# DavidHuji/CapDec

Hardware: AMD Instinct MI355X
Metric: captions/sec (whole node), COCO-val 5k, prefix_len=10 beam=5, 1/2/4/8 GPUs (higher is better)
Workload: dtype f32 (operands split into 2 fp16 planes, 3 fp16 MFMAs per product, fp32 accumulate); 1 GPU; COCO-val-5k-shaped: 5000 x 512-d synthetic CLIP embeddings in total (sharded over the ranks) -> normalise -> TransformerMapper(8 layers) -> GPT-2 small KV-cached beam-5 decode, prefix_len 10, entry_length 67, hot-init seeded weights (never emit the stop id: all 67 steps run); captions_per_gpu=5000, beam=5, parallelism=caption-shard dp1

## Files before the change

### capdec_amd/csrc/bf16x3.h

```cpp
#pragma once
#include <hip/hip_runtime.h>
#include <stdint.h>

namespace capdec {

typedef __bf16 bf16x8 __attribute__((ext_vector_type(8)));
typedef __bf16 bf16x4 __attribute__((ext_vector_type(4)));

constexpr int X3_BK = 16;
constexpr int X3_ROW_B = 32;
constexpr int X3_TILE_ROWS = 128;
constexpr int X3_PLANE_B = X3_TILE_ROWS * X3_ROW_B;
constexpr int X3_BLOCK_B = 3 * X3_PLANE_B;

__device__ __forceinline__ void split3(const float4 v, bf16x4 &h, bf16x4 &m, bf16x4 &l) {
    const float a[4] = {v.x, v.y, v.z, v.w};
#pragma unroll
    for (int e = 0; e < 4; ++e) {
        const __bf16 hh = (__bf16)a[e];
        const float r1 = a[e] - (float)hh;
        const __bf16 mm = (__bf16)r1;
        const float r2 = r1 - (float)mm;
        h[e] = hh;
        m[e] = mm;
        l[e] = (__bf16)r2;
    }
}

__device__ __forceinline__ int x3_group_offset(int r, int quad) {
    return r * X3_ROW_B + (((quad >> 1) ^ ((r >> 3) & 1)) << 4) + ((quad & 1) << 3);
}

typedef _Float16 f16x8 __attribute__((ext_vector_type(8)));
typedef _Float16 f16x4 __attribute__((ext_vector_type(4)));
enum PackFmt { PK_BF16X3 = 0, PK_F16X2 = 1, PK_BF16X1 = 2, PK_F16X1 = 3 };
constexpr int H2_BLOCK_B = 2 * X3_PLANE_B;
constexpr float H2_LO_SCALE = 2048.0f;

static __device__ unsigned int g_h2_saturated;
#define CAPDEC_SAT_ACCESSOR(fn)                                                                            \
    unsigned long long fn(bool reset) {                                                                    \
        unsigned int v = 0;                                                                                \
        if (hipMemcpyFromSymbol(&v, HIP_SYMBOL(g_h2_saturated), sizeof(v)) != hipSuccess) return 0;        \
        if (reset && v) { const unsigned int z = 0; (void)hipMemcpyToSymbol(HIP_SYMBOL(g_h2_saturated), &z, sizeof(z)); } \
        return v;                                                                                          \
    }
__device__ __forceinline__ float h2_clamp_count(const float4 v) {
    const float m = __builtin_fmaxf(__builtin_fmaxf(__builtin_fabsf(v.x), __builtin_fabsf(v.y)),
                                    __builtin_fmaxf(__builtin_fabsf(v.z), __builtin_fabsf(v.w)));
    if (m > 65504.f) atomicAdd(&g_h2_saturated, 1u);
    return m;
}
__device__ __forceinline__ float h2_clamp(float a) {
    return a != a ? a : __builtin_fminf(__builtin_fmaxf(a, -65504.f), 65504.f);
}

__device__ __forceinline__ void split2h(const float4 v, f16x4 &h, f16x4 &l) {
    const float a[4] = {v.x, v.y, v.z, v.w};
    (void)h2_clamp_count(v);
#pragma unroll
    for (int e = 0; e < 4; ++e) {
        const float c = h2_clamp(a[e]);
        const _Float16 hh = __builtin_fabsf(c) < 0x1p-14f ? (_Float16)0.f : (_Float16)c;
        const float r = c - (float)hh;
        h[e] = hh;
        l[e] = (_Float16)(r * H2_LO_SCALE);
    }
}

__host__ __device__ __forceinline__ int pk_planes(int fmt) {
    return fmt == PK_F16X2 ? 2 : (fmt == PK_BF16X1 || fmt == PK_F16X1) ? 1 : 3;
}

__device__ __forceinline__ void x3_store_quad(char *packed, int nk, int row, int ks, int quad, const float4 v,
                                              int fmt = PK_BF16X3) {
    if (fmt == PK_BF16X1 || fmt == PK_F16X1) {
        char *p = packed + ((size_t)(row >> 7) * nk + ks) * X3_PLANE_B + x3_group_offset(row & 127, quad);
        if (fmt == PK_BF16X1) {
            bf16x4 h;
            h[0] = (__bf16)v.x; h[1] = (__bf16)v.y; h[2] = (__bf16)v.z; h[3] = (__bf16)v.w;
            *reinterpret_cast<bf16x4 *>(p) = h;
        } else {
            f16x4 h;
            (void)h2_clamp_count(v);
            h[0] = (_Float16)h2_clamp(v.x);
            h[1] = (_Float16)h2_clamp(v.y);
            h[2] = (_Float16)h2_clamp(v.z);
            h[3] = (_Float16)h2_clamp(v.w);
            *reinterpret_cast<f16x4 *>(p) = h;
        }
        return;
    }
    if (fmt == PK_F16X2) {
        f16x4 h, l;
        split2h(v, h, l);
        char *p = packed + ((size_t)(row >> 7) * nk + ks) * H2_BLOCK_B + x3_group_offset(row & 127, quad);
        *reinterpret_cast<f16x4 *>(p) = h;
        *reinterpret_cast<f16x4 *>(p + X3_PLANE_B) = l;
        return;
    }
    bf16x4 h, m, l;
    split3(v, h, m, l);
    char *p = packed + ((size_t)(row >> 7) * nk + ks) * X3_BLOCK_B + x3_group_offset(row & 127, quad);
    *reinterpret_cast<bf16x4 *>(p) = h;
    *reinterpret_cast<bf16x4 *>(p + X3_PLANE_B) = m;
    *reinterpret_cast<bf16x4 *>(p + 2 * X3_PLANE_B) = l;
}

__device__ __forceinline__ float4 x3_load_quad(const char *packed, int nk, int row, int ks, int quad, int fmt) {
    if (fmt == PK_F16X2) {
        const char *p = packed + ((size_t)(row >> 7) * nk + ks) * H2_BLOCK_B + x3_group_offset(row & 127, quad);
        const f16x4 h = *reinterpret_cast<const f16x4 *>(p), l = *reinterpret_cast<const f16x4 *>(p + X3_PLANE_B);
        return make_float4((float)h[0] + (float)l[0] * (1.0f / H2_LO_SCALE), (float)h[1] + (float)l[1] * (1.0f / H2_LO_SCALE),
                           (float)h[2] + (float)l[2] * (1.0f / H2_LO_SCALE), (float)h[3] + (float)l[3] * (1.0f / H2_LO_SCALE));
    }
    const char *p = packed + ((size_t)(row >> 7) * nk + ks) * X3_PLANE_B + x3_group_offset(row & 127, quad);
    if (fmt == PK_F16X1) {
        const f16x4 h = *reinterpret_cast<const f16x4 *>(p);
        return make_float4((float)h[0], (float)h[1], (float)h[2], (float)h[3]);
    }
    const bf16x4 h = *reinterpret_cast<const bf16x4 *>(p);
    return make_float4((float)h[0], (float)h[1], (float)h[2], (float)h[3]);
}

inline size_t x3_packed_bytes(int rows, int K, int fmt = PK_BF16X3) {
    return (size_t)((rows + X3_TILE_ROWS - 1) / X3_TILE_ROWS) * X3_TILE_ROWS * K * pk_planes(fmt) * sizeof(uint16_t);
}

}
```

### capdec_amd/csrc/elementwise.hip

```cpp
#include "bf16x3.h"
#include "common.h"

namespace capdec {

constexpr int LN_MAXV = 4;
__global__ __launch_bounds__(256) void layernorm_kernel(const float *__restrict__ x, int ldx,
                                                        const float *__restrict__ w, const float *__restrict__ b,
                                                        float eps, float *__restrict__ y, int ldy, int rows, int d) {
    const int lane = threadIdx.x & 63;
    const int row = blockIdx.x * 4 + (threadIdx.x >> 6);
    if (row >= rows) return;
    const float *xr = x + (size_t)row * ldx;
    const int nv = d >> 2;
    float4 v[LN_MAXV];
    float s = 0.f;
#pragma unroll
    for (int i = 0; i < LN_MAXV; ++i) {
        const int idx = lane + 64 * i;
        if (idx < nv) {
            v[i] = reinterpret_cast<const float4 *>(xr)[idx];
            s += (v[i].x + v[i].y) + (v[i].z + v[i].w);
        } else {
            v[i] = make_float4(0.f, 0.f, 0.f, 0.f);
        }
    }
    const float mean = wave_sum(s) / (float)d;
    float q = 0.f;
#pragma unroll
    for (int i = 0; i < LN_MAXV; ++i) {
        const int idx = lane + 64 * i;
        if (idx < nv) {
            const float a = v[i].x - mean, bb = v[i].y - mean, c = v[i].z - mean, e = v[i].w - mean;
            q += (a * a + bb * bb) + (c * c + e * e);
        }
    }
    const float rstd = 1.0f / sqrtf(wave_sum(q) / (float)d + eps);
    float *yr = y + (size_t)row * ldy;
#pragma unroll
    for (int i = 0; i < LN_MAXV; ++i) {
        const int idx = lane + 64 * i;
        if (idx < nv) {
            const float4 ww = reinterpret_cast<const float4 *>(w)[idx];
            const float4 bb = reinterpret_cast<const float4 *>(b)[idx];
            float4 o;
            o.x = (v[i].x - mean) * rstd * ww.x + bb.x;
            o.y = (v[i].y - mean) * rstd * ww.y + bb.y;
            o.z = (v[i].z - mean) * rstd * ww.z + bb.z;
            o.w = (v[i].w - mean) * rstd * ww.w + bb.w;
            reinterpret_cast<float4 *>(yr)[idx] = o;
        }
    }
}

int launch_layernorm(hipStream_t st, const float *x, int ldx, const float *w, const float *b, float eps, float *y,
                     int ldy, int rows, int d) {
    CAPDEC_CHECK(d % 4 == 0 && d <= 256 * LN_MAXV && ldx % 4 == 0 && ldy % 4 == 0, "layernorm: unsupported width");
    if (rows <= 0) return 0;
    hipLaunchKernelGGL(layernorm_kernel, dim3((rows + 3) / 4), dim3(256), 0, st, x, ldx, w, b, eps, y, ldy, rows, d);
    CAPDEC_HIP(hipGetLastError());
    return 0;
}

template <int LN_RPW>
__global__ __launch_bounds__(256) void layernorm_packed_kernel(const float *__restrict__ x, int ldx,
                                                               const float *__restrict__ w, const float *__restrict__ b,
                                                               float eps, char *__restrict__ packed, int rows, int d,
                                                               int fmt) {
    const int lane = threadIdx.x & 63, wave = threadIdx.x >> 6;
    const int nv = d >> 2, nk = d / X3_BK;
    const int row0 = blockIdx.x * 4 * LN_RPW + wave;
    if (row0 >= rows) return;
    float4 ww[LN_MAXV], bb[LN_MAXV];
#pragma unroll
    for (int i = 0; i < LN_MAXV; ++i) {
        const int idx = lane + 64 * i;
        ww[i] = idx < nv ? reinterpret_cast<const float4 *>(w)[idx] : make_float4(0.f, 0.f, 0.f, 0.f);
        bb[i] = idx < nv ? reinterpret_cast<const float4 *>(b)[idx] : make_float4(0.f, 0.f, 0.f, 0.f);
    }
    float4 v[LN_MAXV], nx[LN_MAXV];
#define LN_LOAD(dst, r)                                                                              \
    _Pragma("unroll") for (int i = 0; i < LN_MAXV; ++i) {                                            \
        const int idx = lane + 64 * i;                                                               \
        dst[i] = (idx < nv && (r) < rows) ? reinterpret_cast<const float4 *>(x + (size_t)(r) * ldx)[idx] \
                                          : make_float4(0.f, 0.f, 0.f, 0.f);                         \
    }
    LN_LOAD(nx, row0)
#pragma unroll
    for (int rr = 0; rr < LN_RPW; ++rr) {
        const int row = row0 + 4 * rr;
        if (row >= rows) break;
#pragma unroll
        for (int i = 0; i < LN_MAXV; ++i) v[i] = nx[i];
        if (rr + 1 < LN_RPW) { LN_LOAD(nx, row + 4) }
        float s = 0.f;
#pragma unroll
        for (int i = 0; i < LN_MAXV; ++i) s += (v[i].x + v[i].y) + (v[i].z + v[i].w);
        const float mean = wave_sum(s) / (float)d;
        float q = 0.f;
#pragma unroll
        for (int i = 0; i < LN_MAXV; ++i) {
            const int idx = lane + 64 * i;
            if (idx < nv) {
                const float a = v[i].x - mean, b2 = v[i].y - mean, c = v[i].z - mean, e = v[i].w - mean;
                q += (a * a + b2 * b2) + (c * c + e * e);
            }
        }
        const float rstd = 1.0f / sqrtf(wave_sum(q) / (float)d + eps);
#pragma unroll
        for (int i = 0; i < LN_MAXV; ++i) {
            const int idx = lane + 64 * i;
            if (idx < nv) {
                float4 o;
                o.x = (v[i].x - mean) * rstd * ww[i].x + bb[i].x;
                o.y = (v[i].y - mean) * rstd * ww[i].y + bb[i].y;
                o.z = (v[i].z - mean) * rstd * ww[i].z + bb[i].z;
                o.w = (v[i].w - mean) * rstd * ww[i].w + bb[i].w;
                x3_store_quad(packed, nk, row, idx >> 2, idx & 3, o, fmt);
            }
        }
    }
#undef LN_LOAD
}

int launch_layernorm_packed(hipStream_t st, const float *x, int ldx, const float *w, const float *b, float eps,
                            void *packed, int rows, int d, int fmt) {
    CAPDEC_CHECK(d % 16 == 0 && d <= 256 * LN_MAXV && ldx % 4 == 0, "layernorm_packed: unsupported width");
    if (rows <= 0) return 0;
    if (rows >= 16384)
        hipLaunchKernelGGL(layernorm_packed_kernel<4>, dim3((rows + 15) / 16), dim3(256), 0, st, x, ldx, w, b, eps,
                           (char *)packed, rows, d, fmt);
    else
        hipLaunchKernelGGL(layernorm_packed_kernel<1>, dim3((rows + 3) / 4), dim3(256), 0, st, x, ldx, w, b, eps,
                           (char *)packed, rows, d, fmt);
    CAPDEC_HIP(hipGetLastError());
    return 0;
}

template <int LN_RPW>
__global__ __launch_bounds__(256) void l2norm_rows_kernel(const float *__restrict__ x, char *__restrict__ packed,
                                                          float *__restrict__ y, int rows, int d, int fmt,
                                                          int *__restrict__ row_bad, int *__restrict__ any_bad) {
    const int lane = threadIdx.x & 63, wave = threadIdx.x >> 6;
    const int nv = d >> 2, nk = d / X3_BK;
    const int row0 = blockIdx.x * 4 * LN_RPW + wave;
    if (row0 >= rows) return;
    float4 v[LN_MAXV], nx[LN_MAXV];
#define L2_LOAD(dst, r)                                                                              \
    _Pragma("unroll") for (int i = 0; i < LN_MAXV; ++i) {                                            \
        const int idx = lane + 64 * i;                                                               \
        dst[i] = (idx < nv && (r) < rows) ? reinterpret_cast<const float4 *>(x + (size_t)(r) * d)[idx] \
                                          : make_float4(0.f, 0.f, 0.f, 0.f);                         \
    }
    L2_LOAD(nx, row0)
#pragma unroll
    for (int rr = 0; rr < LN_RPW; ++rr) {
        const int row = row0 + 4 * rr;
        if (row >= rows) break;
#pragma unroll
        for (int i = 0; i < LN_MAXV; ++i) v[i] = nx[i];
        if (rr + 1 < LN_RPW) { L2_LOAD(nx, row + 4) }
        float q = 0.f, big = 0.f;
#pragma unroll
        for (int i = 0; i < LN_MAXV; ++i) {
            q += (v[i].x * v[i].x + v[i].y * v[i].y) + (v[i].z * v[i].z + v[i].w * v[i].w);
            const float a = __builtin_fabsf(v[i].x), b = __builtin_fabsf(v[i].y), c = __builtin_fabsf(v[i].z),
                        e = __builtin_fabsf(v[i].w);
            big = (a <= 3.402823466e38f && b <= 3.402823466e38f && c <= 3.402823466e38f && e <= 3.402823466e38f) ? big : 1.f;
        }
        const bool bad = wave_max(big) != 0.f;
        const float den = fmaxf(sqrtf(wave_sum(q)), 1e-12f);
        if (lane == 0) {
            if (row_bad) row_bad[row] = bad ? 1 : 0;
            if (bad && any_bad) atomicOr(any_bad, 1);
        }
#pragma unroll
        for (int i = 0; i < LN_MAXV; ++i) {
            const int idx = lane + 64 * i;
            if (idx < nv) {
                const float4 o = bad ? make_float4(0.f, 0.f, 0.f, 0.f)
                                     : make_float4(v[i].x / den, v[i].y / den, v[i].z / den, v[i].w / den);
                if (packed) x3_store_quad(packed, nk, row, idx >> 2, idx & 3, o, fmt);
                else reinterpret_cast<float4 *>(y + (size_t)row * d)[idx] = o;
            }
        }
    }
#undef L2_LOAD
}

int launch_l2norm_rows(hipStream_t st, const float *x, void *packed, float *y, int rows, int d, int fmt, int *row_bad,
                       int *any_bad) {
    CAPDEC_CHECK(d % 4 == 0 && d <= 256 * LN_MAXV && (!packed || d % 16 == 0), "l2norm_rows: unsupported width");
    CAPDEC_CHECK((packed != nullptr) != (y != nullptr), "l2norm_rows: exactly one output form");
    if (rows <= 0) return 0;
    if (rows >= 16384)
        hipLaunchKernelGGL(l2norm_rows_kernel<4>, dim3((rows + 15) / 16), dim3(256), 0, st, x, (char *)packed, y, rows, d, fmt,
                           row_bad, any_bad);
    else
        hipLaunchKernelGGL(l2norm_rows_kernel<1>, dim3((rows + 3) / 4), dim3(256), 0, st, x, (char *)packed, y, rows, d, fmt,
                           row_bad, any_bad);
    CAPDEC_HIP(hipGetLastError());
    return 0;
}

__global__ void embed_tokens_kernel(const int *__restrict__ tok, const float *__restrict__ wte,
                                    const float *__restrict__ wpe_row, float *__restrict__ h, int rows, int nv,
                                    const int *__restrict__ cmap, int beam) {
    const int i = blockIdx.x * blockDim.x + threadIdx.x;
    if (i >= rows * nv) return;
    const int row = i / nv, c = i - row * nv;
    const int srow = cmap ? cmap[row / beam] * beam + row % beam : row;
    const float4 a = reinterpret_cast<const float4 *>(wte + (size_t)tok[srow] * nv * 4)[c];
    const float4 p = reinterpret_cast<const float4 *>(wpe_row)[c];
    reinterpret_cast<float4 *>(h)[i] = make_float4(a.x + p.x, a.y + p.y, a.z + p.z, a.w + p.w);
}
int launch_embed_tokens(hipStream_t st, const int *tok, const float *wte, const float *wpe_row, float *h, int rows,
                        int d, const int *cmap, int beam) {
    if (rows <= 0) return 0;
    const int n = rows * (d / 4);
    hipLaunchKernelGGL(embed_tokens_kernel, dim3((n + 255) / 256), dim3(256), 0, st, tok, wte, wpe_row, h, rows,
                       d / 4, cmap, beam);
    CAPDEC_HIP(hipGetLastError());
    return 0;
}

__global__ void embed_prefix_kernel(const float *__restrict__ prefix, const float *__restrict__ wpe,
                                    float *__restrict__ h, int n, int P, int pos0, int nv) {
    const int i = blockIdx.x * blockDim.x + threadIdx.x;
    if (i >= n * P * nv) return;
    const int c = i % nv, p = (i / nv) % P;
    const float4 a = reinterpret_cast<const float4 *>(prefix)[i];
    const float4 w = reinterpret_cast<const float4 *>(wpe + (size_t)(pos0 + p) * nv * 4)[c];
    reinterpret_cast<float4 *>(h)[i] = make_float4(a.x + w.x, a.y + w.y, a.z + w.z, a.w + w.w);
}
int launch_embed_prefix(hipStream_t st, const float *prefix, const float *wpe, float *h, int n, int P, int pos0,
                        int d) {
    const int tot = n * P * (d / 4);
    if (tot <= 0) return 0;
    hipLaunchKernelGGL(embed_prefix_kernel, dim3((tot + 255) / 256), dim3(256), 0, st, prefix, wpe, h, n, P, pos0,
                       d / 4);
    CAPDEC_HIP(hipGetLastError());
    return 0;
}

__global__ void gather_rows_kernel(const float *__restrict__ table, const int *__restrict__ ids,
                                   float *__restrict__ out, int rows, int nv) {
    const int i = blockIdx.x * blockDim.x + threadIdx.x;
    if (i >= rows * nv) return;
    const int row = i / nv, c = i - row * nv;
    reinterpret_cast<float4 *>(out)[i] = reinterpret_cast<const float4 *>(table + (size_t)ids[row] * nv * 4)[c];
}
int launch_gather_rows(hipStream_t st, const float *table, const int *ids, float *out, int rows, int d) {
    if (rows <= 0) return 0;
    const int n = rows * (d / 4);
    hipLaunchKernelGGL(gather_rows_kernel, dim3((n + 255) / 256), dim3(256), 0, st, table, ids, out, rows, d / 4);
    CAPDEC_HIP(hipGetLastError());
    return 0;
}

__global__ __launch_bounds__(256) void normalize_prefix_kernel(const float *__restrict__ x, int n, int dim,
                                                               int normalize, const float *__restrict__ offset,
                                                               float *__restrict__ out) {
    const int lane = threadIdx.x & 63;
    const int row = blockIdx.x * 4 + (threadIdx.x >> 6);
    if (row >= n) return;
    const float *xr = x + (size_t)row * dim;
    float s = 0.f;
    for (int i = lane; i < dim; i += 64) s += xr[i] * xr[i];
    const float nrm = sqrtf(wave_sum(s));
    for (int i = lane; i < dim; i += 64) {
        float v = xr[i];
        if (normalize) v = v / nrm;
        if (offset) v += offset[i];
        out[(size_t)row * dim + i] = v;
    }
}
int launch_normalize_prefix(hipStream_t st, const float *x, int n, int dim, int normalize, const float *offset,
                            float *out) {
    if (n <= 0) return 0;
    hipLaunchKernelGGL(normalize_prefix_kernel, dim3((n + 3) / 4), dim3(256), 0, st, x, n, dim, normalize, offset,
                       out);
    CAPDEC_HIP(hipGetLastError());
    return 0;
}

__device__ __forceinline__ float u01(uint32_t x) { return ((float)(x >> 8) + 0.5f) * (1.0f / 16777216.0f); }
__device__ __forceinline__ float philox_normal(uint64_t seed, uint64_t idx, uint32_t stream) {
    uint32_t o[4];
    philox4x32((uint32_t)idx, (uint32_t)(idx >> 32), stream, 0u, (uint32_t)seed, (uint32_t)(seed >> 32), o);
    const float r = sqrtf(-2.0f * logf(u01(o[0])));
    return r * cosf(6.283185307179586f * u01(o[1]));
}
__device__ __forceinline__ float philox_uniform(uint64_t seed, uint64_t idx, uint32_t stream) {
    uint32_t o[4];
    philox4x32((uint32_t)idx, (uint32_t)(idx >> 32), stream, 0u, (uint32_t)seed, (uint32_t)(seed >> 32), o);
    return ((float)(o[0] >> 8)) * (1.0f / 16777216.0f);
}

__global__ __launch_bounds__(256) void noise_inject_kernel(const float *__restrict__ x, int n, int dim, float std,
                                                           const float *__restrict__ offset, int uniform,
                                                           int dont_norm, uint64_t seed,
                                                           const float *__restrict__ noise,
                                                           const float *__restrict__ u, float *__restrict__ out) {
    const int lane = threadIdx.x & 63;
    const int row = blockIdx.x * 4 + (threadIdx.x >> 6);
    if (row >= n) return;
    const float *xr = x + (size_t)row * dim;
    float inv1 = 1.f;
    if (!dont_norm) {
        float s = 0.f;
        for (int i = lane; i < dim; i += 64) s += xr[i] * xr[i];
        inv1 = 1.0f / fmaxf(sqrtf(wave_sum(s)), 1e-12f);
    }
    float nscale = std;
    if (uniform) {
        float s = 0.f;
        for (int i = lane; i < dim; i += 64) {
            const float g = noise ? noise[(size_t)row * dim + i] : philox_normal(seed, (uint64_t)row * dim + i, 0u);
            s += g * g;
        }
        const float gn = fmaxf(sqrtf(wave_sum(s)), 1e-12f);
        const float uu = u ? u[row] : philox_uniform(seed, (uint64_t)row, 1u);
        nscale = powf(uu, 1.0f / (float)dim) * std / gn;
    }
    float s2 = 0.f;
    for (int i = lane; i < dim; i += 64) {
        const float g = noise ? noise[(size_t)row * dim + i] : philox_normal(seed, (uint64_t)row * dim + i, 0u);
        float v = (dont_norm ? xr[i] : xr[i] * inv1);
        v = v + g * nscale;
        if (offset) v += offset[i];
        out[(size_t)row * dim + i] = v;
        s2 += v * v;
    }
    const float inv2 = 1.0f / fmaxf(sqrtf(wave_sum(s2)), 1e-12f);
    for (int i = lane; i < dim; i += 64) out[(size_t)row * dim + i] *= inv2;
}
int launch_noise_inject(hipStream_t st, const float *x, int n, int dim, float variance, const float *offset,
                        int uniform, int dont_norm, uint64_t seed, const float *noise, const float *u, float *out) {
    if (n <= 0) return 0;
    if (variance == 0.0f) {
        if (out != x) CAPDEC_HIP(hipMemcpyAsync(out, x, (size_t)n * dim * sizeof(float), hipMemcpyDeviceToDevice, st));
        return 0;
    }
    CAPDEC_CHECK(out != x, "noise_inject: in-place not supported");
    hipLaunchKernelGGL(noise_inject_kernel, dim3((n + 3) / 4), dim3(256), 0, st, x, n, dim, sqrtf(variance), offset,
                       uniform, dont_norm, seed, noise, u, out);
    CAPDEC_HIP(hipGetLastError());
    return 0;
}

__global__ void tmapper_concat_kernel(const float *__restrict__ lin, const float *__restrict__ pc,
                                      float *__restrict__ seq, int n, int clip_len, int P, int nv) {
    const int i = blockIdx.x * blockDim.x + threadIdx.x;
    const int S = clip_len + P;
    if (i >= n * S * nv) return;
    const int c = i % nv, s = (i / nv) % S, cap = i / (nv * S);
    float4 v;
    if (s < clip_len) v = reinterpret_cast<const float4 *>(lin)[((size_t)cap * clip_len + s) * nv + c];
    else v = reinterpret_cast<const float4 *>(pc)[(size_t)(s - clip_len) * nv + c];
    reinterpret_cast<float4 *>(seq)[i] = v;
}
int launch_tmapper_concat(hipStream_t st, const float *lin, const float *prefix_const, float *seq, int n,
                          int clip_len, int P, int d) {
    const int tot = n * (clip_len + P) * (d / 4);
    if (tot <= 0) return 0;
    hipLaunchKernelGGL(tmapper_concat_kernel, dim3((tot + 255) / 256), dim3(256), 0, st, lin, prefix_const, seq, n,
                       clip_len, P, d / 4);
    CAPDEC_HIP(hipGetLastError());
    return 0;
}
__global__ void tmapper_take_kernel(const float *__restrict__ seq, float *__restrict__ out, int n, int clip_len,
                                    int P, int nv) {
    const int i = blockIdx.x * blockDim.x + threadIdx.x;
    if (i >= n * P * nv) return;
    const int c = i % nv, p = (i / nv) % P, cap = i / (nv * P);
    reinterpret_cast<float4 *>(out)[i] =
        reinterpret_cast<const float4 *>(seq)[((size_t)cap * (clip_len + P) + clip_len + p) * nv + c];
}
int launch_tmapper_take(hipStream_t st, const float *seq, float *out, int n, int clip_len, int P, int d) {
    const int tot = n * P * (d / 4);
    if (tot <= 0) return 0;
    hipLaunchKernelGGL(tmapper_take_kernel, dim3((tot + 255) / 256), dim3(256), 0, st, seq, out, n, clip_len, P,
                       d / 4);
    CAPDEC_HIP(hipGetLastError());
    return 0;
}

__global__ void transpose_kernel(const float *__restrict__ in, float *__restrict__ out, int rows, int cols) {
    __shared__ float tile[32][33];
    const int bx = blockIdx.x * 32, by = blockIdx.y * 32;
    const int tx = threadIdx.x & 31, ty = threadIdx.x >> 5;
    for (int j = ty; j < 32; j += 8) {
        const int r = by + j, c = bx + tx;
        if (r < rows && c < cols) tile[j][tx] = in[(size_t)r * cols + c];
    }
    __syncthreads();
    for (int j = ty; j < 32; j += 8) {
        const int c = bx + j, r = by + tx;
        if (r < rows && c < cols) out[(size_t)c * rows + r] = tile[tx][j];
    }
}
int launch_transpose(hipStream_t st, const float *in, float *out, int rows, int cols) {
    hipLaunchKernelGGL(transpose_kernel, dim3((cols + 31) / 32, (rows + 31) / 32), dim3(256), 0, st, in, out, rows,
                       cols);
    CAPDEC_HIP(hipGetLastError());
    return 0;
}

__global__ void clip_text_embed_kernel(const int *__restrict__ tokens, const float *__restrict__ tok_emb,
                                       const float *__restrict__ pos_emb, float *__restrict__ h, int n, int L, int P,
                                       const int *__restrict__ perm, int nv) {
    const int i = blockIdx.x * blockDim.x + threadIdx.x;
    if (i >= n * P * nv) return;
    const int c = i % nv, row = i / nv, t = row % P, cap = row / P;
    const int tok = tokens[(size_t)(perm ? perm[cap] : cap) * L + t];
    const float4 a = reinterpret_cast<const float4 *>(tok_emb + (size_t)tok * nv * 4)[c];
    const float4 p = reinterpret_cast<const float4 *>(pos_emb + (size_t)t * nv * 4)[c];
    reinterpret_cast<float4 *>(h)[i] = make_float4(a.x + p.x, a.y + p.y, a.z + p.z, a.w + p.w);
}
int launch_clip_text_embed(hipStream_t st, const int *tokens, const float *tok_emb, const float *pos_emb, float *h,
                           int n, int L, int d, int P, const int *perm) {
    if (P <= 0) P = L;
    const int tot = n * P * (d / 4);
    if (tot <= 0) return 0;
    hipLaunchKernelGGL(clip_text_embed_kernel, dim3((tot + 255) / 256), dim3(256), 0, st, tokens, tok_emb, pos_emb, h, n,
                       L, P, perm, d / 4);
    CAPDEC_HIP(hipGetLastError());
    return 0;
}

__global__ void eot_index_kernel(const int *__restrict__ tokens, int *__restrict__ flat_idx, int n, int L, int flat) {
    const int r = blockIdx.x * blockDim.x + threadIdx.x;
    if (r >= n) return;
    int best = tokens[(size_t)r * L], bi = 0;
    for (int t = 1; t < L; ++t) {
        const int v = tokens[(size_t)r * L + t];
        if (v > best) { best = v; bi = t; }
    }
    flat_idx[r] = (flat ? r * L : 0) + bi;
}
int launch_eot_index(hipStream_t st, const int *tokens, int *flat_idx, int n, int L, int flat) {
    if (n <= 0) return 0;
    hipLaunchKernelGGL(eot_index_kernel, dim3((n + 255) / 256), dim3(256), 0, st, tokens, flat_idx, n, L, flat);
    CAPDEC_HIP(hipGetLastError());
    return 0;
}
__global__ void eot_rows_kernel(const int *__restrict__ pos, const int *__restrict__ perm, int *__restrict__ rows, int m, int P) {
    const int i = blockIdx.x * blockDim.x + threadIdx.x;
    if (i < m) rows[i] = i * P + pos[perm[i]];
}
int launch_eot_rows(hipStream_t st, const int *pos, const int *perm, int *rows, int m, int P) {
    if (m <= 0) return 0;
    hipLaunchKernelGGL(eot_rows_kernel, dim3((m + 255) / 256), dim3(256), 0, st, pos, perm, rows, m, P);
    CAPDEC_HIP(hipGetLastError());
    return 0;
}
__global__ void scatter_rows_kernel(const float *__restrict__ src, const int *__restrict__ perm, float *__restrict__ dst, int rows, int nv) {
    const int i = blockIdx.x * blockDim.x + threadIdx.x;
    if (i >= rows * nv) return;
    const int row = i / nv, c = i - row * nv;
    reinterpret_cast<float4 *>(dst + (size_t)perm[row] * nv * 4)[c] = reinterpret_cast<const float4 *>(src)[i];
}
int launch_scatter_rows(hipStream_t st, const float *src, const int *perm, float *dst, int rows, int d) {
    if (rows <= 0) return 0;
    const int n = rows * (d / 4);
    hipLaunchKernelGGL(scatter_rows_kernel, dim3((n + 255) / 256), dim3(256), 0, st, src, perm, dst, rows, d / 4);
    CAPDEC_HIP(hipGetLastError());
    return 0;
}

__global__ void im2col_patches_kernel(const float *__restrict__ pixels, float *__restrict__ patches, int n, int S,
                                      int patch) {
    const int g = S / patch, kq = patch / 4;
    const size_t i = (size_t)blockIdx.x * blockDim.x + threadIdx.x;
    const size_t tot = (size_t)n * g * g * 3 * patch * kq;
    if (i >= tot) return;
    const int x4 = i % kq;
    size_t r = i / kq;
    const int ky = r % patch; r /= patch;
    const int c = r % 3; r /= 3;
    const int px = r % g; r /= g;
    const int py = r % g;
    const int img = r / g;
    const float4 v = *reinterpret_cast<const float4 *>(
        pixels + (((size_t)img * 3 + c) * S + (py * patch + ky)) * S + px * patch + x4 * 4);
    reinterpret_cast<float4 *>(patches)[i] = v;
}
int launch_im2col_patches(hipStream_t st, const float *pixels, float *patches, int n, int S, int patch) {
    CAPDEC_CHECK(S % patch == 0 && patch % 4 == 0, "im2col: bad patch geometry");
    const int g = S / patch;
    const size_t tot = (size_t)n * g * g * 3 * patch * (patch / 4);
    if (tot == 0) return 0;
    hipLaunchKernelGGL(im2col_patches_kernel, dim3((unsigned)((tot + 255) / 256)), dim3(256), 0, st, pixels, patches, n,
                       S, patch);
    CAPDEC_HIP(hipGetLastError());
    return 0;
}

__global__ void vision_assemble_kernel(const float *__restrict__ patch_out, const float *__restrict__ cls,
                                       const float *__restrict__ pos, float *__restrict__ seq, int n, int ntok,
                                       int nv) {
    const int i = blockIdx.x * blockDim.x + threadIdx.x;
    if (i >= n * ntok * nv) return;
    const int c = i % nv, t = (i / nv) % ntok, img = i / (nv * ntok);
    const float4 p = reinterpret_cast<const float4 *>(pos)[(size_t)t * nv + c];
    const float4 a = t == 0 ? reinterpret_cast<const float4 *>(cls)[c]
                            : reinterpret_cast<const float4 *>(patch_out)[((size_t)img * (ntok - 1) + t - 1) * nv + c];
    reinterpret_cast<float4 *>(seq)[i] = make_float4(a.x + p.x, a.y + p.y, a.z + p.z, a.w + p.w);
}
int launch_vision_assemble(hipStream_t st, const float *patch_out, const float *cls, const float *pos, float *seq,
                           int n, int ntok, int d) {
    const int tot = n * ntok * (d / 4);
    if (tot <= 0) return 0;
    hipLaunchKernelGGL(vision_assemble_kernel, dim3((tot + 255) / 256), dim3(256), 0, st, patch_out, cls, pos, seq, n,
                       ntok, d / 4);
    CAPDEC_HIP(hipGetLastError());
    return 0;
}

template <int PLANES>
__global__ __launch_bounds__(256) void gather_packed_rows_kernel(const char *__restrict__ packed, int nk,
                                                                 const int *__restrict__ src_rows,
                                                                 const int *__restrict__ count_dev, char *__restrict__ out) {
    constexpr int BLOCK_B = PLANES * X3_PLANE_B;
    const int lane = threadIdx.x & 63;
    const int n = *count_dev;
    for (int i = blockIdx.x * 4 + (threadIdx.x >> 6); i < n; i += gridDim.x * 4) {
        const int r = src_rows[i];
        for (int q = lane; q < nk * 4; q += 64) {
            const int ks = q >> 2, quad = q & 3;
            const char *sp = packed + ((size_t)(r >> 7) * nk + ks) * BLOCK_B + x3_group_offset(r & 127, quad);
            char *dp = out + ((size_t)(i >> 7) * nk + ks) * BLOCK_B + x3_group_offset(i & 127, quad);
#pragma unroll
            for (int pl = 0; pl < PLANES; ++pl)
                *reinterpret_cast<uint2 *>(dp + pl * X3_PLANE_B) = *reinterpret_cast<const uint2 *>(sp + pl * X3_PLANE_B);
        }
    }
}
int launch_gather_packed_rows(hipStream_t st, const void *packed, int K, const int *src_rows, const int *count_dev,
                              int rows_cap, void *out, int fmt) {
    CAPDEC_CHECK(K % 16 == 0 && rows_cap > 0, "gather_packed_rows: bad sizes");
    CAPDEC_CHECK(fmt == PK_F16X2 || fmt == PK_F16X1 || fmt == PK_BF16X1, "gather_packed_rows: f16x2 or one-plane operands");
    const dim3 grid(std::min((rows_cap + 3) / 4, 1024));
    if (fmt == PK_F16X2)
        hipLaunchKernelGGL(gather_packed_rows_kernel<2>, grid, dim3(256), 0, st, (const char *)packed, K / X3_BK, src_rows,
                           count_dev, (char *)out);
    else
        hipLaunchKernelGGL(gather_packed_rows_kernel<1>, grid, dim3(256), 0, st, (const char *)packed, K / X3_BK, src_rows,
                           count_dev, (char *)out);
    CAPDEC_HIP(hipGetLastError());
    return 0;
}

CAPDEC_SAT_ACCESSOR(sat_count_elementwise)

}
```

### capdec_amd/csrc/gemm_epilogue_lds.h

```cpp
#pragma once
#include "gemm_epilogue.h"

namespace capdec {

struct EpiArgs {
    float *C = nullptr;
    int ldc = 0, M = 0, N = 0, m0 = 0, n0 = 0;
    const float *bias = nullptr;
    const float *resid = nullptr;
    int ldr = 0, act = CAPDEC_ACT_NONE;
    float scale = 1.0f;
    char *packed = nullptr;
    const char *resid_pk = nullptr;
    int fmt = PK_F16X2;
    const QkvScatter *sc = nullptr;
};

template <int TJ> struct EpiSlab {
    static constexpr int W = TJ * 32, LD = W + 4;
    static constexpr int BYTES = 32 * LD * 4;
};

template <int ACT> __device__ __forceinline__ float act_const(float v) {
    if constexpr (ACT == CAPDEC_ACT_TANH) return tanhf(v);
    else if constexpr (ACT == CAPDEC_ACT_RELU) return fmaxf(v, 0.f);
    else if constexpr (ACT == CAPDEC_ACT_GELU_NEW) {
        const float c2 = 2.0f * 0.7978845608028654f;
        const float u2 = v * (c2 + (c2 * 0.044715f) * v * v);
        return __fdividef(v, 1.f + __expf(-u2));
    } else if constexpr (ACT == CAPDEC_ACT_QUICK_GELU) return __fdividef(v, 1.f + __expf(-1.702f * v));
    else return v;
}
template <int ACT> __device__ __forceinline__ float post_resid_const(float v) {
    if constexpr (ACT == CAPDEC_ACT_RESID_RELU) return fmaxf(v, 0.f);
    else return v;
}

template <int TJ, int Q> struct EpiWalk {
    static constexpr int LPR = TJ * 8 / Q;
    static constexpr int PASSES = (32 * LPR + 63) / 64;
};

template <int TI, int TJ, int MODE, int ACT, bool AHEAD = false>
__device__ __forceinline__ void epilogue_lds_wave(const f32x16 (&acc)[TI][TJ], float *slab, int row0, int col0,
                                                  const EpiArgs &a) {
    using S = EpiSlab<TJ>;
    const int lane = threadIdx.x & 63, half = lane >> 5, l32 = lane & 31;
    constexpr int Q = MODE == 1 ? 2 : 1;
    using Wk = EpiWalk<TJ, Q>;
    constexpr bool PRE = AHEAD && MODE != 1;
    static_assert(!PRE || (64 % Wk::LPR == 0 && Wk::PASSES * 64 == 32 * Wk::LPR), "AHEAD: one column per lane, whole passes");
    float4 bq = make_float4(0.f, 0.f, 0.f, 0.f);
    float4 rq[PRE && MODE == 0 ? TI * Wk::PASSES : 1];
    if constexpr (PRE) {
        const int colc = min(col0 + (lane % Wk::LPR) * 4, a.N - 4);
        if (a.bias) bq = *reinterpret_cast<const float4 *>(a.bias + colc);
        if constexpr (MODE == 0) {
            if (a.resid) {
#pragma unroll
                for (int i = 0; i < TI; ++i)
#pragma unroll
                    for (int p = 0; p < Wk::PASSES; ++p) {
                        const int rowc = min(row0 + i * 32 + (p * 64 + lane) / Wk::LPR, a.M - 1);
                        rq[i * Wk::PASSES + p] = *reinterpret_cast<const float4 *>(a.resid + (size_t)rowc * a.ldr + colc);
                    }
            }
        }
    }
#pragma unroll
    for (int i = 0; i < TI; ++i) {
#pragma unroll
        for (int j = 0; j < TJ; ++j)
#pragma unroll
            for (int g = 0; g < 4; ++g)
                *reinterpret_cast<float4 *>(slab + l32 * S::LD + j * 32 + 8 * g + 4 * half) = acc_quad(acc[i][j], g);
        __builtin_amdgcn_fence(__ATOMIC_RELEASE, "wavefront");
        __builtin_amdgcn_wave_barrier();
        __builtin_amdgcn_fence(__ATOMIC_ACQUIRE, "wavefront");
#pragma unroll
        for (int p = 0; p < Wk::PASSES; ++p) {
            const int idx = p * 64 + lane;
            const int rl = idx / Wk::LPR, cq = idx - rl * Wk::LPR;
            const int row = row0 + i * 32 + rl, col = col0 + cq * (4 * Q);
            const bool live = (Wk::PASSES * 64 == 32 * Wk::LPR || rl < 32) && row < a.M && col < a.N;
            if (!live) continue;
            float4 v[Q];
#pragma unroll
            for (int q = 0; q < Q; ++q) {
                v[q] = *reinterpret_cast<const float4 *>(slab + rl * S::LD + cq * (4 * Q) + 4 * q);
                v[q].x *= a.scale; v[q].y *= a.scale; v[q].z *= a.scale; v[q].w *= a.scale;
                if (a.bias) {
                    float4 b;
                    if constexpr (PRE) b = bq;
                    else b = *reinterpret_cast<const float4 *>(a.bias + col + 4 * q);
                    v[q].x += b.x; v[q].y += b.y; v[q].z += b.z; v[q].w += b.w;
                }
                v[q].x = act_const<ACT>(v[q].x); v[q].y = act_const<ACT>(v[q].y);
                v[q].z = act_const<ACT>(v[q].z); v[q].w = act_const<ACT>(v[q].w);
            }
            if constexpr (MODE == 0) {
                if (a.resid) {
                    float4 r4;
                    if constexpr (PRE) r4 = rq[i * Wk::PASSES + p];
                    else r4 = *reinterpret_cast<const float4 *>(a.resid + (size_t)row * a.ldr + col);
                    v[0].x = post_resid_const<ACT>(v[0].x + r4.x); v[0].y = post_resid_const<ACT>(v[0].y + r4.y);
                    v[0].z = post_resid_const<ACT>(v[0].z + r4.z); v[0].w = post_resid_const<ACT>(v[0].w + r4.w);
                }
                *reinterpret_cast<float4 *>(a.C + (size_t)row * a.ldc + col) = v[0];
            } else if constexpr (MODE == 2) {
                const QkvScatter &sc = *a.sc;
                if (col < sc.d) {
                    *reinterpret_cast<float4 *>(a.C + (size_t)row * a.ldc + col) = v[0];
                } else {
                    const int cap = row / sc.beam, b = row - cap * sc.beam;
                    const size_t srow = (size_t)(sc.cmap ? sc.cmap[cap] : cap) * sc.beam + b;
                    float *cache = col >= 2 * sc.d ? sc.vc : sc.kc;
                    const int hc = col - (col >= 2 * sc.d ? 2 * sc.d : sc.d), head = hc >> 6;
                    const size_t el = ((srow * sc.heads + head) * sc.ctx + sc.pos) * 64 + (hc & 63);
                    if (sc.bf16) {
                        bf16x4 t;
                        t[0] = (__bf16)v[0].x; t[1] = (__bf16)v[0].y; t[2] = (__bf16)v[0].z; t[3] = (__bf16)v[0].w;
                        *reinterpret_cast<bf16x4 *>(reinterpret_cast<__bf16 *>(cache) + el) = t;
                    } else
                        *reinterpret_cast<float4 *>(cache + el) = v[0];
                }
            } else {
                const int nk_out = a.N >> 4, ks = col >> 4, hf = (col >> 3) & 1, r7 = row & 127;
                const size_t blk = (size_t)(row >> 7) * nk_out + ks;
                const int inrow = r7 * X3_ROW_B + ((hf ^ ((r7 >> 3) & 1)) << 4);
                if (a.resid_pk) {
#pragma unroll
                    for (int q = 0; q < Q; ++q) {
                        const float4 rr = x3_load_quad(a.resid_pk, nk_out, row, ks, 2 * hf + q, a.fmt);
                        v[q].x = post_resid_const<ACT>(v[q].x + rr.x); v[q].y = post_resid_const<ACT>(v[q].y + rr.y);
                        v[q].z = post_resid_const<ACT>(v[q].z + rr.z); v[q].w = post_resid_const<ACT>(v[q].w + rr.w);
                    }
                }
                if (a.fmt == PK_F16X2) {
                    f16x4 h0, l0, h1, l1;
                    split2h(v[0], h0, l0);
                    split2h(v[1], h1, l1);
                    char *pp = a.packed + blk * H2_BLOCK_B + inrow;
                    f16x8 hh, ll;
#pragma unroll
                    for (int e = 0; e < 4; ++e) { hh[e] = h0[e]; hh[4 + e] = h1[e]; ll[e] = l0[e]; ll[4 + e] = l1[e]; }
                    *reinterpret_cast<f16x8 *>(pp) = hh;
                    *reinterpret_cast<f16x8 *>(pp + X3_PLANE_B) = ll;
                } else {
                    x3_store_quad(a.packed, nk_out, row, ks, 2 * hf, v[0], a.fmt);
                    x3_store_quad(a.packed, nk_out, row, ks, 2 * hf + 1, v[1], a.fmt);
                }
            }
        }
        __builtin_amdgcn_fence(__ATOMIC_RELEASE, "wavefront");
        __builtin_amdgcn_wave_barrier();
        __builtin_amdgcn_fence(__ATOMIC_ACQUIRE, "wavefront");
    }
}

template <int TI, int TJ, int MODE, bool AHEAD = false>
__device__ __forceinline__ void epilogue_lds_dispatch(const f32x16 (&acc)[TI][TJ], float *slab, int row0, int col0,
                                                      const EpiArgs &a) {
    switch (a.act) {
        case CAPDEC_ACT_GELU_NEW: epilogue_lds_wave<TI, TJ, MODE, CAPDEC_ACT_GELU_NEW, AHEAD>(acc, slab, row0, col0, a); break;
        case CAPDEC_ACT_QUICK_GELU: epilogue_lds_wave<TI, TJ, MODE, CAPDEC_ACT_QUICK_GELU, AHEAD>(acc, slab, row0, col0, a); break;
        case CAPDEC_ACT_RELU: epilogue_lds_wave<TI, TJ, MODE, CAPDEC_ACT_RELU, AHEAD>(acc, slab, row0, col0, a); break;
        case CAPDEC_ACT_TANH: epilogue_lds_wave<TI, TJ, MODE, CAPDEC_ACT_TANH, AHEAD>(acc, slab, row0, col0, a); break;
        case CAPDEC_ACT_RESID_RELU: epilogue_lds_wave<TI, TJ, MODE, CAPDEC_ACT_RESID_RELU, AHEAD>(acc, slab, row0, col0, a); break;
        default: epilogue_lds_wave<TI, TJ, MODE, CAPDEC_ACT_NONE, AHEAD>(acc, slab, row0, col0, a); break;
    }
}

template <class G, bool AHEAD = false>
__device__ __forceinline__ void epilogue_lds(const f32x16 (&acc)[G::TI][G::TJ], char *smem, const EpiArgs &a) {
    const int wave = __builtin_amdgcn_readfirstlane(threadIdx.x >> 6);
    const int wm = wave / G::WN, wn = wave % G::WN;
    float *slab = reinterpret_cast<float *>(smem + wave * EpiSlab<G::TJ>::BYTES);
    const int row0 = a.m0 + wm * G::TI * 32, col0 = a.n0 + wn * G::TJ * 32;
    if (a.packed) epilogue_lds_dispatch<G::TI, G::TJ, 1>(acc, slab, row0, col0, a);
    else if (a.sc && a.sc->kc) epilogue_lds_wave<G::TI, G::TJ, 2, CAPDEC_ACT_NONE, AHEAD>(acc, slab, row0, col0, a);
    else epilogue_lds_dispatch<G::TI, G::TJ, 0, AHEAD>(acc, slab, row0, col0, a);
}

}
```

Baseline: 3035 captions/s.

## Add specialized interior epilogues for fp16x2 packing and QKV scatter, plus line-packed layernorm

Adds a fast-path GEMM epilogue for interior tiles writing fp16x2 packed output. It skips bounds checks, batches the saturation counter into one atomic per wave, and skips clamping when no lane saturates. It also adds a specialized QKV-to-KV-cache scatter epilogue that precomputes caption map indices, and a layernorm-to-packed kernel that uses 16 lanes per row with weights staged in LDS. Together these target per-element branching, atomics and index arithmetic in memory-bound epilogues, at the cost of more code paths and template instantiations.

New measurement: 3084 captions/s (median of 6 runs). +1.6%, better.

```diff
diff --git a/capdec_amd/csrc/bf16x3.h b/capdec_amd/csrc/bf16x3.h
--- a/capdec_amd/csrc/bf16x3.h
+++ b/capdec_amd/csrc/bf16x3.h
@@ -55,12 +55,22 @@
     return a != a ? a : __builtin_fminf(__builtin_fmaxf(a, -65504.f), 65504.f);
 }
 
+__device__ __forceinline__ unsigned int h2_saturates(const float4 v) {
+    const float m = __builtin_fmaxf(__builtin_fmaxf(__builtin_fabsf(v.x), __builtin_fabsf(v.y)),
+                                    __builtin_fmaxf(__builtin_fabsf(v.z), __builtin_fabsf(v.w)));
+    return m > 65504.f ? 1u : 0u;
+}
+__device__ __forceinline__ void h2_post_saturated(unsigned int n) {
+    if (n) atomicAdd(&g_h2_saturated, n);
+}
+
+template <bool COUNTED = true, bool CLAMP = true>
 __device__ __forceinline__ void split2h(const float4 v, f16x4 &h, f16x4 &l) {
     const float a[4] = {v.x, v.y, v.z, v.w};
-    (void)h2_clamp_count(v);
+    if constexpr (COUNTED) (void)h2_clamp_count(v);
 #pragma unroll
     for (int e = 0; e < 4; ++e) {
-        const float c = h2_clamp(a[e]);
+        const float c = CLAMP ? h2_clamp(a[e]) : a[e];
         const _Float16 hh = __builtin_fabsf(c) < 0x1p-14f ? (_Float16)0.f : (_Float16)c;
         const float r = c - (float)hh;
         h[e] = hh;
diff --git a/capdec_amd/csrc/elementwise.hip b/capdec_amd/csrc/elementwise.hip
--- a/capdec_amd/csrc/elementwise.hip
+++ b/capdec_amd/csrc/elementwise.hip
@@ -122,11 +122,69 @@
 #undef LN_LOAD
 }
 
+template <int NJ>
+__global__ __launch_bounds__(256) void layernorm_packed_lines_kernel(const float *__restrict__ x, int ldx,
+                                                                     const float *__restrict__ w, const float *__restrict__ b,
+                                                                     float eps, char *__restrict__ packed, int rows, int d,
+                                                                     int fmt) {
+    __shared__ float4 sw[NJ * 16], sb[NJ * 16];
+    const int lane = threadIdx.x & 63, wave = threadIdx.x >> 6, g = lane >> 4, t = lane & 15;
+    const int nv = d >> 2, nj = nv >> 4, nk = d / X3_BK;
+    const int row = (blockIdx.x * 4 + wave) * 4 + g;
+    float4 v[NJ];
+#pragma unroll
+    for (int j = 0; j < NJ; ++j)
+        v[j] = (j < nj && row < rows) ? reinterpret_cast<const float4 *>(x + (size_t)row * ldx)[16 * j + t]
+                                      : make_float4(0.f, 0.f, 0.f, 0.f);
+    for (int i = threadIdx.x; i < nv; i += 256) {
+        sw[i] = reinterpret_cast<const float4 *>(w)[i];
+        sb[i] = reinterpret_cast<const float4 *>(b)[i];
+    }
+    __syncthreads();
+    float s[4] = {0.f, 0.f, 0.f, 0.f};
+#pragma unroll
+    for (int i = 0; i < LN_MAXV; ++i)
+#pragma unroll
+        for (int m = 0; m < 4; ++m) {
+            const int j = 4 * i + m;
+            if (j < NJ && j < nj) s[m] += (v[j].x + v[j].y) + (v[j].z + v[j].w);
+        }
+    const float mean = ((row16_sum(s[0]) + row16_sum(s[1])) + (row16_sum(s[2]) + row16_sum(s[3]))) / (float)d;
+    float q[4] = {0.f, 0.f, 0.f, 0.f};
+#pragma unroll
+    for (int i = 0; i < LN_MAXV; ++i)
+#pragma unroll
+        for (int m = 0; m < 4; ++m) {
+            const int j = 4 * i + m;
+            if (j < NJ && j < nj) {
+                const float a = v[j].x - mean, b2 = v[j].y - mean, c = v[j].z - mean, e = v[j].w - mean;
+                q[m] += (a * a + b2 * b2) + (c * c + e * e);
+            }
+        }
+    const float rstd = 1.0f / sqrtf(((row16_sum(q[0]) + row16_sum(q[1])) + (row16_sum(q[2]) + row16_sum(q[3]))) / (float)d + eps);
+#pragma unroll
+    for (int j = 0; j < NJ; ++j) {
+        if (j < nj && row < rows) {
+            const int idx = 16 * j + t;
+            const float4 ww = sw[idx], bb = sb[idx];
+            float4 o;
+            o.x = (v[j].x - mean) * rstd * ww.x + bb.x;
+            o.y = (v[j].y - mean) * rstd * ww.y + bb.y;
+            o.z = (v[j].z - mean) * rstd * ww.z + bb.z;
+            o.w = (v[j].w - mean) * rstd * ww.w + bb.w;
+            x3_store_quad(packed, nk, row, idx >> 2, idx & 3, o, fmt);
+        }
+    }
+}
+
 int launch_layernorm_packed(hipStream_t st, const float *x, int ldx, const float *w, const float *b, float eps,
                             void *packed, int rows, int d, int fmt) {
     CAPDEC_CHECK(d % 16 == 0 && d <= 256 * LN_MAXV && ldx % 4 == 0, "layernorm_packed: unsupported width");
     if (rows <= 0) return 0;
-    if (rows >= 16384)
+    if (rows >= 16384 && d % 64 == 0 && d <= 768)
+        hipLaunchKernelGGL(layernorm_packed_lines_kernel<12>, dim3((rows + 15) / 16), dim3(256), 0, st, x, ldx, w, b, eps,
+                           (char *)packed, rows, d, fmt);
+    else if (rows >= 16384)
         hipLaunchKernelGGL(layernorm_packed_kernel<4>, dim3((rows + 15) / 16), dim3(256), 0, st, x, ldx, w, b, eps,
                            (char *)packed, rows, d, fmt);
     else
diff --git a/capdec_amd/csrc/gemm_epilogue_lds.h b/capdec_amd/csrc/gemm_epilogue_lds.h
--- a/capdec_amd/csrc/gemm_epilogue_lds.h
+++ b/capdec_amd/csrc/gemm_epilogue_lds.h
@@ -158,9 +158,170 @@
     }
 }
 
+template <int TI, int TJ> __device__ __forceinline__ void epilogue_slab_fill(const f32x16 (&acc)[TI][TJ], float *slab, int i) {
+    using S = EpiSlab<TJ>;
+    const int lane = threadIdx.x & 63, half = lane >> 5, l32 = lane & 31;
+#pragma unroll
+    for (int j = 0; j < TJ; ++j)
+#pragma unroll
+        for (int g = 0; g < 4; ++g)
+            *reinterpret_cast<float4 *>(slab + l32 * S::LD + j * 32 + 8 * g + 4 * half) = acc_quad(acc[i][j], g);
+}
+__device__ __forceinline__ void epilogue_slab_sync() {
+    __builtin_amdgcn_fence(__ATOMIC_RELEASE, "wavefront");
+    __builtin_amdgcn_wave_barrier();
+    __builtin_amdgcn_fence(__ATOMIC_ACQUIRE, "wavefront");
+}
+
+
+template <int TI, int TJ, int ACT>
+__device__ __forceinline__ void epilogue_lds_wave_h2_interior(const f32x16 (&acc)[TI][TJ], float *slab, int row0, int col0,
+                                                              const EpiArgs &a) {
+    using S = EpiSlab<TJ>;
+    using Wk = EpiWalk<TJ, 2>;
+    static_assert(64 % Wk::LPR == 0 && Wk::PASSES * 64 == 32 * Wk::LPR, "one column per lane, whole passes");
+    constexpr int RPP = 64 / Wk::LPR;
+    const int lane = threadIdx.x & 63;
+    const int rl0 = lane / Wk::LPR, cq = lane % Wk::LPR;
+    const int col = col0 + cq * 8;
+    const int nk_out = a.N >> 4, ks = col >> 4, hf = (col >> 3) & 1;
+    const bool has_bias = a.bias != nullptr;
+    float4 b0 = make_float4(0.f, 0.f, 0.f, 0.f), b1 = b0;
+    if (has_bias) {
+        b0 = *reinterpret_cast<const float4 *>(a.bias + col);
+        b1 = *reinterpret_cast<const float4 *>(a.bias + col + 4);
+    }
+    const float *sp = slab + rl0 * S::LD + cq * 8;
+    unsigned int nsat = 0;
+#pragma unroll
+    for (int i = 0; i < TI; ++i) {
+        epilogue_slab_fill<TI, TJ>(acc, slab, i);
+        epilogue_slab_sync();
+        const int rb = row0 + i * 32;
+        char *pb = a.packed + ((size_t)(rb >> 7) * nk_out + ks) * H2_BLOCK_B + ((rb & 96) + rl0) * X3_ROW_B;
+#pragma unroll
+        for (int p = 0; p < Wk::PASSES; ++p) {
+            float4 v[2];
+#pragma unroll
+            for (int q = 0; q < 2; ++q) {
+                v[q] = *reinterpret_cast<const float4 *>(sp + p * RPP * S::LD + 4 * q);
+                v[q].x *= a.scale; v[q].y *= a.scale; v[q].z *= a.scale; v[q].w *= a.scale;
+                if (has_bias) {
+                    const float4 b = q ? b1 : b0;
+                    v[q].x += b.x; v[q].y += b.y; v[q].z += b.z; v[q].w += b.w;
+                }
+                v[q].x = act_const<ACT>(v[q].x); v[q].y = act_const<ACT>(v[q].y);
+                v[q].z = act_const<ACT>(v[q].z); v[q].w = act_const<ACT>(v[q].w);
+            }
+            const unsigned int sat0 = h2_saturates(v[0]), sat1 = h2_saturates(v[1]);
+            nsat += sat0 + sat1;
+            f16x4 h0, l0, h1, l1;
+            if (__builtin_amdgcn_ballot_w64((sat0 | sat1) != 0u)) {
+                split2h<false>(v[0], h0, l0);
+                split2h<false>(v[1], h1, l1);
+            } else {
+                split2h<false, false>(v[0], h0, l0);
+                split2h<false, false>(v[1], h1, l1);
+            }
+            const int sw = ((p * RPP + rl0) >> 3) & 1;
+            char *pp = pb + p * RPP * X3_ROW_B + ((hf ^ sw) << 4);
+            f16x8 hh, ll;
+#pragma unroll
+            for (int e = 0; e < 4; ++e) { hh[e] = h0[e]; hh[4 + e] = h1[e]; ll[e] = l0[e]; ll[4 + e] = l1[e]; }
+            *reinterpret_cast<f16x8 *>(pp) = hh;
+            *reinterpret_cast<f16x8 *>(pp + X3_PLANE_B) = ll;
+        }
+        epilogue_slab_sync();
+    }
+    h2_post_saturated(nsat);
+}
+
+template <int TI, int TJ, bool INTERIOR>
+__device__ __forceinline__ void epilogue_lds_wave_qkv(const f32x16 (&acc)[TI][TJ], float *slab, int row0, int col0,
+                                                      const EpiArgs &a) {
+    using S = EpiSlab<TJ>;
+    using Wk = EpiWalk<TJ, 1>;
+    static_assert(64 % Wk::LPR == 0 && Wk::PASSES * 64 == 32 * Wk::LPR, "one column per lane, whole passes");
+    constexpr int RPP = 64 / Wk::LPR, NP = TI * Wk::PASSES;
+    const QkvScatter &sc = *a.sc;
+    const int lane = threadIdx.x & 63;
+    const int rl0 = lane / Wk::LPR, cq = lane % Wk::LPR;
+    const int col = col0 + cq * 4;
+    const bool col_live = INTERIOR || col < a.N;
+    float4 bq = make_float4(0.f, 0.f, 0.f, 0.f);
+    const bool has_bias = a.bias != nullptr;
+    if (has_bias) bq = *reinterpret_cast<const float4 *>(a.bias + (INTERIOR ? col : min(col, a.N - 4)));
+    const bool is_q = col < sc.d, is_v = col >= 2 * sc.d;
+    float *cache = is_v ? sc.vc : sc.kc;
+    const int hc = col - (is_v ? 2 * sc.d : sc.d), head = hc >> 6;
+    const size_t cell = ((size_t)head * sc.ctx + sc.pos) * 64 + (hc & 63);
+    const size_t row_el = (size_t)sc.heads * sc.ctx * 64;
+    const int beam = sc.beam, step_q = RPP / beam, step_r = RPP - step_q * beam;
+    const int cap0 = (row0 + rl0) / beam, b0 = (row0 + rl0) - cap0 * beam;
+    int cm[NP];
+    {
+        const int cap_last = (a.M - 1) / beam;
+        int cap = cap0, b = b0;
+#pragma unroll
+        for (int k = 0; k < NP; ++k) {
+            cm[k] = sc.cmap ? sc.cmap[INTERIOR ? cap : min(cap, cap_last)] : cap;
+            cap += step_q; b += step_r;
+            if (b >= beam) { b -= beam; ++cap; }
+        }
+    }
+    const float *sp = slab + rl0 * S::LD + cq * 4;
+    int b = b0;
+#pragma unroll
+    for (int i = 0; i < TI; ++i) {
+        epilogue_slab_fill<TI, TJ>(acc, slab, i);
+        epilogue_slab_sync();
+#pragma unroll
+        for (int p = 0; p < Wk::PASSES; ++p) {
+            const int row = row0 + i * 32 + p * RPP + rl0;
+            const int bcur = b;
+            b += step_r;
+            if (b >= beam) b -= beam;
+            if (!INTERIOR && !(col_live && row < a.M)) continue;
+            float4 v = *reinterpret_cast<const float4 *>(sp + p * RPP * S::LD);
+            v.x *= a.scale; v.y *= a.scale; v.z *= a.scale; v.w *= a.scale;
+            if (has_bias) { v.x += bq.x; v.y += bq.y; v.z += bq.z; v.w += bq.w; }
+            if (is_q) {
+                *reinterpret_cast<float4 *>(a.C + (size_t)row * a.ldc + col) = v;
+            } else {
+                const size_t srow = (size_t)cm[i * Wk::PASSES + p] * beam + bcur;
+                const size_t el = srow * row_el + cell;
+                if (sc.bf16) {
+                    bf16x4 t;
+                    t[0] = (__bf16)v.x; t[1] = (__bf16)v.y; t[2] = (__bf16)v.z; t[3] = (__bf16)v.w;
+                    *reinterpret_cast<bf16x4 *>(reinterpret_cast<__bf16 *>(cache) + el) = t;
+                } else
+                    *reinterpret_cast<float4 *>(cache + el) = v;
+            }
+        }
+        epilogue_slab_sync();
+    }
+}
+
+template <int TI, int TJ>
+__device__ __forceinline__ bool epilogue_interior(int row0, int col0, const EpiArgs &a) {
+    return (row0 & 31) == 0 && row0 + TI * 32 <= a.M && col0 + TJ * 32 <= a.N;
+}
+
 template <int TI, int TJ, int MODE, bool AHEAD = false>
 __device__ __forceinline__ void epilogue_lds_dispatch(const f32x16 (&acc)[TI][TJ], float *slab, int row0, int col0,
                                                       const EpiArgs &a) {
+    if constexpr (MODE == 1 && 64 % EpiWalk<TJ, 2>::LPR == 0 && EpiWalk<TJ, 2>::PASSES * 64 == 32 * EpiWalk<TJ, 2>::LPR) {
+        if (a.fmt == PK_F16X2 && !a.resid_pk && epilogue_interior<TI, TJ>(row0, col0, a)) {
+            switch (a.act) {
+                case CAPDEC_ACT_GELU_NEW: epilogue_lds_wave_h2_interior<TI, TJ, CAPDEC_ACT_GELU_NEW>(acc, slab, row0, col0, a); break;
+                case CAPDEC_ACT_QUICK_GELU: epilogue_lds_wave_h2_interior<TI, TJ, CAPDEC_ACT_QUICK_GELU>(acc, slab, row0, col0, a); break;
+                case CAPDEC_ACT_RELU: epilogue_lds_wave_h2_interior<TI, TJ, CAPDEC_ACT_RELU>(acc, slab, row0, col0, a); break;
+                case CAPDEC_ACT_TANH: epilogue_lds_wave_h2_interior<TI, TJ, CAPDEC_ACT_TANH>(acc, slab, row0, col0, a); break;
+                default: epilogue_lds_wave_h2_interior<TI, TJ, CAPDEC_ACT_NONE>(acc, slab, row0, col0, a); break;
+            }
+            return;
+        }
+    }
     switch (a.act) {
         case CAPDEC_ACT_GELU_NEW: epilogue_lds_wave<TI, TJ, MODE, CAPDEC_ACT_GELU_NEW, AHEAD>(acc, slab, row0, col0, a); break;
         case CAPDEC_ACT_QUICK_GELU: epilogue_lds_wave<TI, TJ, MODE, CAPDEC_ACT_QUICK_GELU, AHEAD>(acc, slab, row0, col0, a); break;
@@ -178,8 +339,13 @@
     float *slab = reinterpret_cast<float *>(smem + wave * EpiSlab<G::TJ>::BYTES);
     const int row0 = a.m0 + wm * G::TI * 32, col0 = a.n0 + wn * G::TJ * 32;
     if (a.packed) epilogue_lds_dispatch<G::TI, G::TJ, 1>(acc, slab, row0, col0, a);
-    else if (a.sc && a.sc->kc) epilogue_lds_wave<G::TI, G::TJ, 2, CAPDEC_ACT_NONE, AHEAD>(acc, slab, row0, col0, a);
-    else epilogue_lds_dispatch<G::TI, G::TJ, 0, AHEAD>(acc, slab, row0, col0, a);
-}
-
-}
+    else if (a.sc && a.sc->kc) {
+        if constexpr (AHEAD) {
+            if (epilogue_interior<G::TI, G::TJ>(row0, col0, a)) epilogue_lds_wave_qkv<G::TI, G::TJ, true>(acc, slab, row0, col0, a);
+            else epilogue_lds_wave_qkv<G::TI, G::TJ, false>(acc, slab, row0, col0, a);
+        } else
+            epilogue_lds_wave<G::TI, G::TJ, 2, CAPDEC_ACT_NONE, AHEAD>(acc, slab, row0, col0, a);
+    } else epilogue_lds_dispatch<G::TI, G::TJ, 0, AHEAD>(acc, slab, row0, col0, a);
+}
+
+}
```
